# tgale96/sputnik

Hardware: AMD Instinct MI355X
Metric: effective TFLOP/s (nnz-FLOPs) DSD block=128 M=K=N=4096 @ 1/2/4/8 GPU vs density (higher is better)
Workload: dtype f16

## Files before the change

sputnik_amd/csrc/dispatch.cpp:

```cpp
#include <algorithm>
#include <cstdint>
#include <mutex>

#include "api_internal.h"
#include "block_gemm.h"
#include "dispatch_internal.h"
#include "dsd4w.h"
#include "metadata.h"
#include "sputnik/sputnik.h"
#include "sputnik_amd.h"

namespace sputnik_amd {

static unsigned long long *g_debug = nullptr;

static bool PairsEnabled() {
#ifdef SPUTNIK_NO_PAIRS
  return false;
#endif
  return Knob(kKnobPairs) != 0;
}

#ifndef SPUTNIK_PAIR_MIN_MEAN4
#define SPUTNIK_PAIR_MIN_MEAN4 8
// ... 421 lines not shown
  if (out == OutMode::kAccF32) p.c_ld *= 2;
  if (!acc) p.xcd_rows = Knob(kKnobXcdRows);
  PreparePairs(&p, blocks, stream, dry, !acc);
  GemmParams t = p;
  r->tall = UseTall(&t);
  if (r->tall && !acc && !dds && UseTallPipe(p, blocks, row_max, ta, tb)) {
    p.persistent = 0;
    p.num_jtiles = p.j_limit / 512;
    p.tall_flush_w = Knob(kKnobTallFlushW);
    p.tall_odd_share = Knob(kKnobTallOddShare);
    int dev = 0;
    p.num_tiles = hipGetDevice(&dev) == hipSuccess ? DeviceCUs(dev) : 0;
    r->code = 4;
    r->epi = 7;
    return;
  }
  if (r->tall) {
    p = t;
    BindTileCounter(&p, stream, dry);
  }
  const long long blocks4w = Dsd4wForced() ? (1LL << 40) : blocks;
  if (acc || !Dsd4wEnabled() ||
      !(dds ? Dds4wApplies(p, blocks4w, tb, !ta, true, r->tall)
            : Dsd4wApplies(p, blocks4w, !ta, tb, false, r->tall))) {
    r->code = r->tall ? 2 : p.pair != 0 && p.pair_split > 1 ? 3 : 0;
    return;
  }
  r->code = 1;
  r->epi = Dsd4wEpi();
  if (dds) {
    if (p.pair_xcd2 != 0) p.pair_xcd2 = Knob(kKnobDdsXcd2);
  } else if (Knob(kKnobDsd4w) == 1 && blocks < 12LL * p.num_rows) {
    r->epi = 5;
  }
}

constexpr long long kDsdBtMinRatio = 15000;
static bool BtAppliesDsd(const BlockMatrix &a, bool ta, const Matrix &b, bool tb) {
  if (!tb || ta || !BtGate(b)) return false;
  const long long blocks = a.nonzeros / (kBlock * kBlock);
  return blocks * 16384 >= kDsdBtMinRatio * b.cols;
}

static DenseRoute RouteDsd(const BlockMatrix &a, bool ta, const Matrix &b, bool tb,
                           const Matrix &c, hipStream_t stream, OutMode out, bool dry,
                           BtView view) {
  DenseRoute r;
  r.status = PrepareDsd(a, ta, b, tb, c, &r.p, &r.needs_meta);
  if (r.status != Status::kOk) return r;
  r.bt = out == OutMode::kStore && view != BtView::kOff && BtAppliesDsd(a, ta, b, tb) &&
         BtViewOpen(view, stream);
  if (!r.bt)
    RouteDenseOut(&r, false, a.nonzeros / (kBlock * kBlock),
                  ((long long)a.cols + kBlock - 1) / kBlock, ta, tb, stream, out, dry);
  return r;
}

static DenseRoute RouteDds(const Matrix &a, bool ta, const BlockMatrix &b, bool tb,
                           const Matrix &c, hipStream_t stream, OutMode out, bool dry) {
  DenseRoute r;
  r.status = PrepareDds(a, ta, b, tb, c, &r.p, &r.needs_meta);
  if (r.status == Status::kOk)
    RouteDenseOut(&r, true, b.nonzeros / (kBlock * kBlock), 0, ta, tb, stream, out, dry);
  return r;
}

// ... 408 lines not shown
```

sputnik_amd/csrc/dsd4w.h:

```cpp
#ifndef SPUTNIK_AMD_DSD4W_H_
#define SPUTNIK_AMD_DSD4W_H_

#include <hip/hip_runtime.h>

#include "block_gemm.h"

namespace sputnik_amd {

constexpr int kDsd4wMinMean = 2;
bool Dsd4wApplies(const GemmParams &p, long long blocks, bool s_kc, bool d_kc,
                  bool out_t, bool tall);

hipError_t LaunchDsd4w(int dtype, const GemmParams &p, int epi, bool nt,
                       hipStream_t stream, bool tn = false, bool tt = false);
constexpr int kDsd4wDefaultEpi = 3;

bool Dds4wApplies(const GemmParams &p, long long blocks, bool s_kc, bool d_kc,
                  bool out_t, bool tall);
hipError_t LaunchDds4w(int dtype, const GemmParams &p, int epi, bool nt,
                       hipStream_t stream, bool tn = false, bool tt = false);

bool Sdd4wApplies(const GemmParams &p, bool grouped, bool ta, bool tb, long long blocks = -1);
hipError_t LaunchSdd4w(int dtype, const GemmParams &p, bool ta, bool tb, int epi,
                       hipStream_t stream);

}

#endif
```

sputnik_amd/csrc/dsd4w.hip:

```cpp
#include <hip/hip_runtime.h>
#include <stdint.h>

#include <cstdlib>

#include "api_internal.h"
#include "block_gemm.h"
#include "dsd4w.h"
#include "dsd4w_asm.inc"

namespace sputnik_amd {
namespace {

constexpr int kRankScratch = 24576;
constexpr uint32_t kOob = 0x80000000u;

struct Pick {
  int row_a, row_b, e_a, n_a, e_b, n_b, target;
  int uniform;
};

__device__ Pick rank_wave(const GemmParams &p, char *lds, int wave, int lane,
                          int ra, int rb, int o0_pre, bool pre) {
  const int R = p.num_rows;
  const int o0 = pre ? o0_pre : lane <= R ? p.s_offsets[lane] : 0;
  const int o1 = __shfl_down(o0, 1, 64);
  const int nr = lane < R ? o1 - o0 : -1;
  int *keys = reinterpret_cast<int *>(lds + kRankScratch + wave * 256);
  int *nbr = reinterpret_cast<int *>(lds + kRankScratch + 2048 + wave * 256);
  const bool live = lane < R;
  const int key = live ? (nr << 6) | (63 - lane) : -1;
  keys[lane] = key;
  int4 k4[16];
#pragma unroll
  for (int j = 0; j < 16; ++j) k4[j] = *reinterpret_cast<const int4 *>(keys + 4 * j);
  int rank = 0;
#pragma unroll
  for (int j = 0; j < 16; ++j)
    rank += (k4[j].x > key) + (k4[j].y > key) + (k4[j].z > key) + (k4[j].w > key);
  const unsigned long long ba = __ballot(live && rank == ra);
  const unsigned long long bb = __ballot(live && rank == rb);
  Pick out;
// ... 49 lines not shown
    const int v = i == j ? n_by_rank[i] : (n_by_rank[i] + n_by_rank[j] + 1) / 2;
    atomicMax(&scratch[2], v);
  }
  __syncthreads();
  Pick out;
  out.row_a = __builtin_amdgcn_readfirstlane(scratch[0]);
  out.row_b = __builtin_amdgcn_readfirstlane(scratch[1]);
  out.target = __builtin_amdgcn_readfirstlane(scratch[2]);
  out.uniform = __builtin_amdgcn_readfirstlane(scratch[3]);
  out.e_a = __builtin_amdgcn_readfirstlane(offs[out.row_a]);
  out.n_a = __builtin_amdgcn_readfirstlane(offs[out.row_a + 1]) - out.e_a;
  out.e_b = __builtin_amdgcn_readfirstlane(offs[out.row_b]);
  out.n_b = __builtin_amdgcn_readfirstlane(offs[out.row_b + 1]) - out.e_b;
  __syncthreads();
  return out;
}

__device__ __forceinline__ unsigned long long exp_stamp(int dep) {
#if (SPUTNIK_EXP & 512) != 0
  unsigned long long t;
  asm volatile("s_memrealtime %0\n s_waitcnt lgkmcnt(0)"
               : "=s"(t) : "s"(__builtin_amdgcn_readfirstlane(dep)));
  return t;
#else
  (void)dep;
  return 0;
#endif
}

template <bool kBf16, int kEpi, bool kDds, bool kSdd = false, bool kNt = false,
          bool kTt = false, bool kTn = false>
__global__ void __launch_bounds__(256, 1) dsd4w_kernel(const GemmParams p) {
  constexpr bool kWaveEpi = kEpi != 0;
  constexpr bool kDs = kEpi == 3 || kEpi == 4 || kEpi == 5 || kEpi == 6 || kEpi == 7;
  constexpr bool kBar2 = kEpi == 4;
  constexpr bool kKs = kEpi == 6;
  constexpr bool kTp = kEpi == 7;
  static_assert(!kTp || (!kSdd && !kDds && !kNt && !kTt && !kTn), "tall pipeline: DSD NN");
  static_assert(!kDds || kEpi == 1 || kEpi == 3, "DDS: per-wave epilogue only");
  static_assert(!kSdd || ((kEpi == 3 || (kEpi == 4 && !kTt) || (kEpi == 1 && kTn) ||
                           (kKs && !kNt && !kTt && !kTn)) && !kDds),
                "SDD: double slots (TN: per-step images), per-wave epilogue");
  static_assert(!kKs || kSdd, "K-split: SDD NN only");
  constexpr bool kARowsT = (kTt || kTn) && kSdd;
  constexpr bool kDdsTt = kDds && kTt;
  [[maybe_unused]] const unsigned long long t_entry = __builtin_amdgcn_s_memrealtime();
  __shared__ __attribute__((aligned(1024))) char lds[163840];
  const int tid = threadIdx.x;
  const int lane = tid & 63;
  const int wave = __builtin_amdgcn_readfirstlane(tid >> 6);
  const uint32_t lbase =
      (uint32_t)(uintptr_t)((__attribute__((address_space(3))) char *)lds);

  constexpr int kIdxPreload = 1024;
  const int nb_all = p.s_blocks;
  [[maybe_unused]] const unsigned long long t_karg = exp_stamp(nb_all);
  const bool idx_pre = nb_all <= kIdxPreload &&
                       (reinterpret_cast<uintptr_t>(p.s_indices) & 15) == 0;
  typedef unsigned v4u_t __attribute__((ext_vector_type(4)));
  v4u_t idx_lo = {0u, 0u, 0u, 0u}, idx_hi = {0u, 0u, 0u, 0u};
  if (idx_pre) {
    const __amdgpu_buffer_rsrc_t ri = __builtin_amdgcn_make_buffer_rsrc(
        const_cast<short *>(p.s_indices), 0, (nb_all * 2 + 3) & ~3, 0x00020000);
    idx_lo = __builtin_bit_cast(v4u_t, __builtin_amdgcn_raw_buffer_load_b128(
                                            ri, lane * 32, 0, 0));
    idx_hi = __builtin_bit_cast(v4u_t, __builtin_amdgcn_raw_buffer_load_b128(
                                            ri, lane * 32 + 16, 0, 0));
// ... 725 lines not shown
    } else if constexpr (kSdd && kBar2) {
      if constexpr (kBf16)
        asm volatile(DSD4W_ASM_BF16_W3_SDD : DSD4W_OPERANDS_W : DSD4W_CLOBBERS);
      else
        asm volatile(DSD4W_ASM_F16_W3_SDD : DSD4W_OPERANDS_W : DSD4W_CLOBBERS);
    } else if constexpr (kSdd) {
      if constexpr (kBf16)
        asm volatile(DSD4W_ASM_BF16_W2_SDD : DSD4W_OPERANDS_W : DSD4W_CLOBBERS);
      else
        asm volatile(DSD4W_ASM_F16_W2_SDD : DSD4W_OPERANDS_W : DSD4W_CLOBBERS);
    } else if constexpr (kDds && kDs && (SPUTNIK_EXP & 512) != 0) {
      const unsigned long long t_asm = __builtin_amdgcn_s_memrealtime();
      unsigned long long r0 = 0, r1 = 0, r2 = 0, r3 = 0, r4 = 0;
      if constexpr (kBf16)
        asm volatile(DSD4W_ASM_BF16_W2_DDS_T : [r0] "=&s"(r0), [r1] "=&s"(r1),
                     [r2] "=&s"(r2), [r3] "=&s"(r3), [r4] "=&s"(r4)
                     : DSD4W_INPUTS_W : DSD4W_CLOBBERS);
      else
        asm volatile(DSD4W_ASM_F16_W2_DDS_T : [r0] "=&s"(r0), [r1] "=&s"(r1),
                     [r2] "=&s"(r2), [r3] "=&s"(r3), [r4] "=&s"(r4)
                     : DSD4W_INPUTS_W : DSD4W_CLOBBERS);
      DSD4W_RECORD((unsigned long long)((collect ? 2 : 0) | (producer ? 1 : 0)), 0ull);
    } else if constexpr (kDds && kDs) {
      if constexpr (kBf16)
        asm volatile(DSD4W_ASM_BF16_W2_DDS : DSD4W_OPERANDS_W : DSD4W_CLOBBERS);
      else
        asm volatile(DSD4W_ASM_F16_W2_DDS : DSD4W_OPERANDS_W : DSD4W_CLOBBERS);
    } else if constexpr (kDds) {
      if constexpr (kBf16)
        asm volatile(DSD4W_ASM_BF16_W_DDS : DSD4W_OPERANDS_W : DSD4W_CLOBBERS);
      else
        asm volatile(DSD4W_ASM_F16_W_DDS : DSD4W_OPERANDS_W : DSD4W_CLOBBERS);
    } else if constexpr ((SPUTNIK_EXP & 512) != 0 &&
                         (kEpi == 1 || kEpi == 3 || kEpi == 5)) {
      const unsigned long long t_asm = __builtin_amdgcn_s_memrealtime();
      unsigned long long r0 = 0, r1 = 0, r2 = 0, r3 = 0, r4 = 0;
#define DSD4W_STAMPED(NAME)                                                    \
  asm volatile(NAME : [r0] "=&s"(r0), [r1] "=&s"(r1), [r2] "=&s"(r2),          \
               [r3] "=&s"(r3), [r4] "=&s"(r4)                                  \
               : DSD4W_INPUTS_W : DSD4W_CLOBBERS)
      if constexpr (kEpi == 5) {
        if constexpr (kBf16) DSD4W_STAMPED(DSD4W_ASM_BF16_W4_T);
        else DSD4W_STAMPED(DSD4W_ASM_F16_W4_T);
      } else if constexpr (kEpi == 3) {
        if constexpr (kBf16) DSD4W_STAMPED(DSD4W_ASM_BF16_W2_T);
        else DSD4W_STAMPED(DSD4W_ASM_F16_W2_T);
      } else {
        if constexpr (kBf16) DSD4W_STAMPED(DSD4W_ASM_BF16_W_T);
        else DSD4W_STAMPED(DSD4W_ASM_F16_W_T);
      }
#undef DSD4W_STAMPED
      DSD4W_RECORD((unsigned long long)((collect ? 2 : 0) | (producer ? 1 : 0)), 0ull);
    } else if constexpr (kEpi == 5) {
      if constexpr (kBf16)
        asm volatile(DSD4W_ASM_BF16_W4 : DSD4W_OPERANDS_W : DSD4W_CLOBBERS);
      else
        asm volatile(DSD4W_ASM_F16_W4 : DSD4W_OPERANDS_W : DSD4W_CLOBBERS);
    } else if constexpr (kBar2) {
      if constexpr (kBf16)
        asm volatile(DSD4W_ASM_BF16_W3 : DSD4W_OPERANDS_W : DSD4W_CLOBBERS);
      else
        asm volatile(DSD4W_ASM_F16_W3 : DSD4W_OPERANDS_W : DSD4W_CLOBBERS);
    } else if constexpr (kDs) {
      if constexpr (kBf16)
        asm volatile(DSD4W_ASM_BF16_W2 : DSD4W_OPERANDS_W : DSD4W_CLOBBERS);
      else
        asm volatile(DSD4W_ASM_F16_W2 : DSD4W_OPERANDS_W : DSD4W_CLOBBERS);
    } else if constexpr (kEpi == 2) {
      if constexpr (kBf16)
        asm volatile(DSD4W_ASM_BF16_WL : DSD4W_OPERANDS_W : DSD4W_CLOBBERS);
      else
        asm volatile(DSD4W_ASM_F16_WL : DSD4W_OPERANDS_W : DSD4W_CLOBBERS);
    } else if constexpr (kWaveEpi) {
      if constexpr (kBf16)
        asm volatile(DSD4W_ASM_BF16_W : DSD4W_OPERANDS_W : DSD4W_CLOBBERS);
      else
        asm volatile(DSD4W_ASM_F16_W : DSD4W_OPERANDS_W : DSD4W_CLOBBERS);
    } else {
      if constexpr (kBf16)
        asm volatile(DSD4W_ASM_BF16 : DSD4W_OPERANDS_G : DSD4W_CLOBBERS);
      else
        asm volatile(DSD4W_ASM_F16 : DSD4W_OPERANDS_G : DSD4W_CLOBBERS);
      __syncthreads();
      for (int id = tid; id < 128 * 64; id += 256) {
        const int r = id >> 6, cc = id & 63;
// ... 66 lines not shown

hipError_t LaunchDsd4w(int dtype, const GemmParams &p, int epi, bool nt,
                       hipStream_t stream, bool tn, bool tt) {
  if (p.num_tiles <= 0) return hipSuccess;
  const dim3 grid(p.pair_split == 2 ? p.grid : p.num_tiles), block(256);
  if (tt) {
    if (dtype == 1)
      hipLaunchKernelGGL((dsd4w_kernel<true, 3, false, false, false, true>), grid, block, 0,
                         stream, p);
    else
      hipLaunchKernelGGL((dsd4w_kernel<false, 3, false, false, false, true>), grid, block, 0,
                         stream, p);
    return hipGetLastError();
  }
  if (tn) {
    if (dtype == 1)
      hipLaunchKernelGGL((dsd4w_kernel<true, 1, false, false, false, false, true>), grid,
                         block, 0, stream, p);
    else
      hipLaunchKernelGGL((dsd4w_kernel<false, 1, false, false, false, false, true>), grid,
                         block, 0, stream, p);
    return hipGetLastError();
  }
  if (nt) {
    if (dtype == 1)
      hipLaunchKernelGGL((dsd4w_kernel<true, 3, false, false, true>), grid, block, 0, stream, p);
    else
      hipLaunchKernelGGL((dsd4w_kernel<false, 3, false, false, true>), grid, block, 0, stream, p);
    return hipGetLastError();
  }
#define DSD4W_LAUNCH(B, E) \
  hipLaunchKernelGGL((dsd4w_kernel<B, E, false>), grid, block, 0, stream, p)
  if (dtype == 1) {
    if (epi == 7) DSD4W_LAUNCH(true, 7);
    else if (epi == 5) DSD4W_LAUNCH(true, 5);
    else if (epi == 4) DSD4W_LAUNCH(true, 4);
    else if (epi == 3) DSD4W_LAUNCH(true, 3);
    else if (epi == 2) DSD4W_LAUNCH(true, 2);
    else if (epi == 1) DSD4W_LAUNCH(true, 1);
    else DSD4W_LAUNCH(true, 0);
  } else {
    if (epi == 7) DSD4W_LAUNCH(false, 7);
    else if (epi == 5) DSD4W_LAUNCH(false, 5);
    else if (epi == 4) DSD4W_LAUNCH(false, 4);
    else if (epi == 3) DSD4W_LAUNCH(false, 3);
    else if (epi == 2) DSD4W_LAUNCH(false, 2);
    else if (epi == 1) DSD4W_LAUNCH(false, 1);
    else DSD4W_LAUNCH(false, 0);
  }
#undef DSD4W_LAUNCH
  return hipGetLastError();
}

bool Dds4wApplies(const GemmParams &p, long long blocks, bool s_kc, bool d_kc,
                  bool out_t, bool tall) {
  return out_t && !tall && (s_kc || p.s_block_offsets != nullptr) &&
         (p.pair_split <= 1 || (p.pair_split == 2 && p.split_bn == 512)) &&
         p.persistent == 0 && p.num_rows <= kLptRows &&
         CfgSparse::kBN == 512 && p.j_limit % 128 == 0 &&
         blocks >= (long long)kDsd4wMinMean * p.num_rows;
}

hipError_t LaunchDds4w(int dtype, const GemmParams &p, int epi, bool nt,
                       hipStream_t stream, bool tn, bool tt) {
  if (p.num_tiles <= 0) return hipSuccess;
  const dim3 grid(p.pair_split == 2 ? p.grid : p.num_tiles), block(256);
  if (tt) {
    if (dtype == 1)
      hipLaunchKernelGGL((dsd4w_kernel<true, 3, true, false, false, true>), grid, block, 0,
                         stream, p);
    else
      hipLaunchKernelGGL((dsd4w_kernel<false, 3, true, false, false, true>), grid, block, 0,
                         stream, p);
    return hipGetLastError();
  }
// ... 84 lines not shown
```

sputnik_amd/csrc/gen_dsd4w.py:

```python
import sys

FS = (128, 192)
FD = (160, 224)
SLOT = 8192
DMA_POS = [3, 9, 15, 21, 27, 33, 39, 45, 51, 57]
READS_AT = 2
NAN_F16 = "0x7e007e00"
NAN_BF16 = "0x7fc07fc0"
WAIT_TICKS = 20000000


def mfma(dt, m, n, s, zero_c=False):
    a = 4 * (8 * m + n)
    c = "0" if zero_c else f"a[{a}:{a + 3}]"
    return (f"v_mfma_f32_16x16x32_{dt} a[{a}:{a + 3}], "
            f"v[{FD[s] + 4 * n}:{FD[s] + 4 * n + 3}], "
            f"v[{FS[s] + 4 * m}:{FS[s] + 4 * m + 3}], {c}")


def d_reads(slot, s, into=None):
    out = []
    for n in range(8):
        b = (into or FD)[s] + 4 * n
        out.append(f"ds_read_b64_tr_b16 v[{b}:{b + 1}], %[vrd{n}] offset:{slot * SLOT}")
        out.append(f"ds_read_b64_tr_b16 v[{b + 2}:{b + 3}], %[vrd{n}] "
                   f"offset:{slot * SLOT + 1024}")
    return out


def t_reads(slot, s):
    out = []
    for m in range(8):
        b = FS[s] + 4 * m
        out.append(f"ds_read_b64_tr_b16 v[{b}:{b + 1}], %[vrt{m}] offset:{slot * SLOT}")
        out.append(f"ds_read_b64_tr_b16 v[{b + 2}:{b + 3}], %[vrt{m}] "
                   f"offset:{slot * SLOT + 1024}")
    return out


def s_reads(slot, s):
    return [f"ds_read_b128 v[{FS[s] + 4 * m}:{FS[s] + 4 * m + 3}], %[vrs] "
            f"offset:{slot * SLOT + m * 1024}" for m in range(8)]


def dmas(slot):
    out = []
    for q in range(2):
        out.append((f"s_add_u32 m0, %[ms], {slot * SLOT + q * 1024}",
                    f"buffer_load_dwordx4 %[vs], s[40:43], {'0' if q == 0 else 's72'} "
                    f"offen lds"))
    for q in range(8):
        out.append((f"s_add_u32 m0, %[md], {slot * SLOT + q * 1024}",
                    f"buffer_load_dwordx4 %[vd{(q >> 1) & 1}], s[44:47], s{64 + q} "
                    f"offen lds"))
    return out


VARIANT = {"dds": False, "ds": False, "sdd": False, "nt": False, "tt": False,
           "bar2": False, "tn": False, "ddstt": False, "il": False, "ks": False,
           "tp": False}


def col_order():
    if VARIANT["ddstt"]:
        return False
    return ((VARIANT["dds"] and not VARIANT["nt"])
            or ((VARIANT["tn"] or VARIANT["tt"]) and not VARIANT["sdd"]))


def a_rows_t():
    return (VARIANT["tt"] or VARIANT["tn"]) and VARIANT["sdd"]


def s_block_shift():
    return (24, 8) if VARIANT["sdd"] else (17, 15)


def advance():
    s = ("%[sk32]" if a_rows_t() else
         8192 if VARIANT["dds"] or VARIANT["tn"] else 64)
    return [f"s_add_u32 s40, s40, {s}", "s_addc_u32 s41, s41, 0",
            "s_add_u32 s44, s44, %[k32]", "s_addc_u32 s45, s45, 0"]


def entry_of(xreg, out_reg):
    if VARIANT["tp"]:
        tmp = "s77" if out_reg == "s76" else "s76"
        return ["s_nop 3", f"v_readlane_b32 {out_reg}, %[vent], {xreg}",
                f"v_readlane_b32 {tmp}, %[vent2], {xreg}", f"s_cmp_lt_u32 {xreg}, 64",
                f"s_cselect_b32 {out_reg}, {out_reg}, {tmp}",
                f"s_and_b32 {out_reg}, {out_reg}, 0xffffff"]
    return [f"s_cmp_lt_u32 {xreg}, %[n1]",
            f"s_cselect_b32 {out_reg}, %[b1], %[b2m]",
# ... 334 lines not shown
    k = 2 * (n_odd + n_even)
    check = [f"s_waitcnt vmcnt({k})", "v_readfirstlane_b32 s98, v97",
             "s_cmp_eq_u32 s98, %[epoch]", "s_cbranch_scc0 L_loop_%="]
    loads1 = []
    for f in range(8):
        loads1 += [(4 + 2 * f, x) for x in _pload(f)]
    loads3 = []
    for f in range(8, 24):
        loads3 += [(8 + 2 * (f - 8), x) for x in _pload(f)]
    body = step_ds(dt, 0)
    body += step_ds(dt, 1, wait=n_even, stores=loads1, no_dma=True)
    body += step_ds(dt, 2, wait=8, no_dma=True)
    body += step_ds(dt, 3, wait=-1, stores=loads3, no_dma=True, no_reads=True)
    return flag_load, check, body


def epilogue_collect_pre(cvt):
    out = []
    for f in range(24, 32):
        out += _pload(f)
    for i in range(64):
        t = 224 + 8 * (i % 4)
        out += [f"v_accvgpr_read_b32 v{t + j}, a{4 * i + j}" for j in range(4)]
        out.append(f"s_waitcnt vmcnt({min(31, 63 - i)})")
        p = 96 + 4 * (i % 32)
        out += [f"v_add_f32 v{t + j}, v{t + j}, v{p + j}" for j in range(4)]
        if i + 32 < 64:
            out += _pload(i + 32)
        out += [f"{cvt} v{t + 4}, v{t}, v{t + 1}", f"{cvt} v{t + 5}, v{t + 2}, v{t + 3}",
                f"ds_write_b64 %[vws{i % 8}], v[{t + 4}:{t + 5}] offset:{4096 * (i // 8)}"]
    return out


def prologue_ds():
    out = prologue_setup()

    def issue(pairs):
        r = []
        for m0, ld in pairs:
            r += [m0, "s_nop 0", ld]
        return r
    own_ds = own_ds_dmas if VARIANT["nt"] else (lambda d: [])
    out += issue(per_step_dmas(0)) + advance_per_step()
    out += issue(ds_dmas(0)) + issue(own_ds(0)) + advance_ds()
    out += issue(per_step_dmas(1)) + advance_per_step()
    out += [f"s_waitcnt vmcnt({ds_counts()[1]})", "s_barrier"]
    if VARIANT["ddstt"]:
        out += t_reads(0, 0) + own_reads_kc(0, 0, 0)
    elif VARIANT["nt"]:
        out += own_reads_kc(0, 0, 0) + s_reads_ds(0, 0, 0)
    elif VARIANT["tt"]:
        out += own_reads_kc(0, 0, 0) + d_reads(0, 0, FS)
    else:
        out += d_reads(0, 0) + s_reads_ds(0, 0, 0)
    out += issue(per_step_dmas(2)) + advance_per_step()
    out += issue(ds_dmas(1)) + issue(own_ds(1))
    out.append("s_waitcnt lgkmcnt(0)")
    return out


def convert(cvt, i):
    t = 96 + 8 * (i % 4)
    m, n = i // 8, i % 8
    out = [f"v_accvgpr_read_b32 v{t + j}, a{4 * i + j}" for j in range(4)]
    out += [f"{cvt} v{t + 4}, v{t}, v{t + 1}", f"{cvt} v{t + 5}, v{t + 2}, v{t + 3}",
            f"ds_write_b64 %[vws{n}], v[{t + 4}:{t + 5}] offset:{4096 * m}"]
# ... 76 lines not shown
        base = "%[vw0]" if m < 4 else "%[vw1]"
        off = 16 * (m % 4) * 1040 + 32 * n
        return f"ds_write_b64 {base}, {src} offset:{off}"

    def load(i):
        v = 128 + 4 * (i % 32)
        return [f"s_mov_b32 s78, {(i // 4) * 4096}",
                f"buffer_load_dwordx4 v[{v}:{v + 3}], %[vpl], s[84:87], s78 offen "
                f"offset:{(i % 4) * 1024} sc1"]

    if mode == "nan":
        nan = NAN_F16 if cvt.endswith("f16_f32") else NAN_BF16
        out += [f"v_mov_b32 v96, {nan}", "v_mov_b32 v97, v96"]
        out += [stage(i, "v[96:97]") for i in range(64)]
        return out
    if mode == "collect":
        for i in range(32):
            out += load(i)
    for i in range(64):
        t = 96 + 8 * (i % 4)
        a = 4 * i
        out += [f"v_accvgpr_read_b32 v{t + j}, a{a + j}" for j in range(4)]
        if mode == "collect":
            out.append(f"s_waitcnt vmcnt({min(31, 63 - i)})")
            p = 128 + 4 * (i % 32)
            out += [f"v_add_f32 v{t + j}, v{t + j}, v{p + j}" for j in range(4)]
            if i + 32 < 64:
                out += load(i + 32)
        out += [f"{cvt} v{t + 4}, v{t}, v{t + 1}", f"{cvt} v{t + 5}, v{t + 2}, v{t + 3}"]
        out.append(stage(i, f"v[{t + 4}:{t + 5}]"))
    return out


def epilogue_plain_interleaved(cvt):
    out = ["s_mov_b32 s84, %[cdlo]", "s_mov_b32 s85, %[cdhi]",
           "s_mov_b32 s86, 0x7fffffff", "s_mov_b32 s87, 0x00020000",
           "s_mov_b32 s78, 0"]
    for m in range(8):
        for n in range(8):
            i = 8 * m + n
            t = 96 + 8 * (i % 4)
            out += [f"v_accvgpr_read_b32 v{t + j}, a{4 * i + j}" for j in range(4)]
            out += [f"{cvt} v{t + 4}, v{t}, v{t + 1}", f"{cvt} v{t + 5}, v{t + 2}, v{t + 3}",
                    f"ds_write_b64 %[vws{n}], v[{t + 4}:{t + 5}] offset:{4096 * m}"]
        base = 128 + 16 * (m % 2)
        for j in range(4):
            out.append(f"ds_read_b128 v[{base + 4 * j}:{base + 4 * j + 3}], "
                       f"%[vrb{j}] offset:{4096 * m}")
        out.append("s_waitcnt lgkmcnt(0)")
        for j in range(4):
            out += [f"buffer_store_dwordx4 v[{base + 4 * j}:{base + 4 * j + 3}], %[vco], "
                    f"s[84:87], s78 offen nt",
                    "s_add_u32 s78, s78, %[c4]"]
        out.append("s_nop 1")
    return out


def copy_out():
    out = ["s_waitcnt lgkmcnt(0)",
           "s_mov_b32 s84, %[cdlo]", "s_mov_b32 s85, %[cdhi]",
           "s_mov_b32 s86, 0x7fffffff", "s_mov_b32 s87, 0x00020000",
           "s_mov_b32 s78, 0"]
    for b in range(8):
        base = 96 + 16 * (b % 2)
        idx = [4 * b + j for j in range(4)]
        for j, i in enumerate(idx):
            out.append(f"ds_read_b128 v[{base + 4 * j}:{base + 4 * j + 3}], "
                       f"%[vrb{i % 4}] offset:{4096 * (i // 4)}")
        out.append("s_waitcnt lgkmcnt(0)")
        for j, i in enumerate(idx):
            out += [f"buffer_store_dwordx4 v[{base + 4 * j}:{base + 4 * j + 3}], %[vco], "
                    f"s[84:87], s78 offen nt",
                    "s_add_u32 s78, s78, %[c4]"]
        out.append("s_nop 1")
    return out


def poll():
    return ["s_memrealtime s[96:97]", "s_waitcnt lgkmcnt(0)",
            "L_poll_%=:",
            "v_mov_b32 v96, 0",
            "global_load_dword v97, v96, %[flag] sc1",
            "s_waitcnt vmcnt(0)", "s_nop 0",
            "v_readfirstlane_b32 s98, v97",
            "s_cmp_eq_u32 s98, %[epoch]", "s_cbranch_scc1 L_got_%=",
            "s_sleep 1",
            "s_memrealtime s[98:99]", "s_waitcnt lgkmcnt(0)",
            "s_sub_u32 s98, s98, s96", "s_subb_u32 s99, s99, s97",
            "s_cmp_lg_u32 s99, 0", "s_cbranch_scc1 L_timeout_%=",
            f"s_cmp_lt_u32 s98, {WAIT_TICKS}", "s_cbranch_scc1 L_poll_%=",
            "L_timeout_%=:",
            "s_bitcmp1_b32 %[flags], 4", "s_cbranch_scc0 L_nan_%=",
            "s_mov_b64 s[78:79], exec", "s_mov_b64 exec, 1",
            "v_mov_b32 v96, 0", "v_mov_b32 v97, 1",
            "global_atomic_add v96, v97, %[err]",
            "s_waitcnt vmcnt(0)",
            "s_mov_b64 exec, s[78:79]",
            "s_branch L_nan_%="]


TP_NO_STORES = [False]


def tall_flush(cvt, dt, stamps=False):
    out = ["L_tflush_%=:"]
    if stamps:
# ... 150 lines not shown
    b0, nb = 8 * g // S, 8 // S
    out += ["s_waitcnt lgkmcnt(0)",
            "s_mov_b32 s84, %[cdlo]", "s_mov_b32 s85, %[cdhi]",
            "s_mov_b32 s86, 0x7fffffff", "s_mov_b32 s87, 0x00020000",
            f"s_mul_i32 s78, %[c4], {4 * b0}"]
    for b in range(b0, b0 + nb):
        base = 96 + 16 * (b % 2)
        for j in range(4):
            out.append(f"ds_read_b128 v[{base + 4 * j}:{base + 4 * j + 3}], "
                       f"%[vrb{j}] offset:{4096 * b}")
        out.append("s_waitcnt lgkmcnt(0)")
        for j in range(4):
            out += [f"buffer_store_dwordx4 v[{base + 4 * j}:{base + 4 * j + 3}], %[vco], "
                    f"s[84:87], s78 offen nt",
                    "s_add_u32 s78, s78, %[c4]"]
        out.append("s_nop 1")
    out.append("s_branch L_fin_%=")
    return out


def ksplit():
    out = ["L_ks_%=:"]
    for S in KS_CHUNKS:
        for g in range(S):
            out += [f"s_cmp_eq_u32 %[kss], {S}", f"s_cbranch_scc0 L_ksn{S}_{g}_%=",
                    f"s_cmp_eq_u32 %[kch], {g}", f"s_cbranch_scc1 L_ks{S}_{g}_%=",
                    f"L_ksn{S}_{g}_%=:"]
    out.append("s_branch L_fin_%=")
    return out


def build(dt, wave_epi=False, last_block=False, stamps=False, dds=False, ds=False,
          sdd=False, nt=False, tt=False, bar2=False, tn=False, ddstt=False, il=False,
          ks=False, tp=False):
    VARIANT.update(dds=dds, ds=ds, sdd=sdd, nt=nt, tt=tt, bar2=bar2, tn=tn, ddstt=ddstt,
                   il=il, ks=ks, tp=tp)
    try:
        return _build(dt, wave_epi, last_block, stamps)
    finally:
        VARIANT.update(dds=False, ds=False, sdd=False, nt=False, tt=False, bar2=False,
                       tn=False, ddstt=False, il=False, ks=False, tp=False)


def _build(dt, wave_epi, last_block, stamps):
    cvt = f"v_cvt_pk_{dt}_f32"
    body = prologue()
    if VARIANT["tp"]:
        body.append("s_mov_b32 s90, 0")
    if stamps and VARIANT["tp"]:
        body += ["s_mov_b32 s88, 0", "s_mov_b32 s89, 0"]
    if stamps:
        body.append("s_memrealtime %[r0]")
    body.append("s_branch L_first_%=")
    early = VARIANT["ds"] and not VARIANT["bar2"] and not VARIANT["sdd"]
    body.append("L_loop_%=:")
    body += step(dt, 0)
    body.append("L_mid_%=:")
    for H in (1, 2, 3):
        if H == 2:
            body.append("L_s2_%=:")
        if H == 3:
            if early:
                body += ["s_cmp_eq_u32 s61, %[pubat]", "s_cbranch_scc1 L_pubs_%=",
                         "s_cmp_eq_u32 s61, %[publast]", "s_cbranch_scc1 L_publ_%="]
            body.append("L_s3_%=:")
        body += step(dt, H)
    if VARIANT["tp"]:
        body.append("L_blkend_%=:")
    body.append("s_sub_u32 s61, s61, 1")
    if VARIANT["tp"]:
        body += ["s_sub_u32 s74, %[ntot], s61", "s_sub_u32 s74, s74, 1", "s_nop 3",
                 "v_readlane_b32 s75, %[vtile], s74", "v_readlane_b32 s76, %[vtile2], s74",
                 "s_cmp_lt_u32 s74, 64", "s_cselect_b32 s75, s75, s76",
                 "s_bitcmp1_b32 s75, 31", "s_cbranch_scc1 L_tflush_%="]
    body += ["s_cmp_eq_u32 s61, %[flushrem]", "s_cbranch_scc1 L_pub_%="]
    if early:
        body += ["s_cmp_eq_u32 s61, %[clbf]", "s_cbranch_scc1 L_clbf_%=",
                 "s_cmp_eq_u32 s61, %[clbc]", "s_cbranch_scc1 L_clbc_%="]
    if last_block:
        body += ["s_cmp_eq_u32 s61, 1", "s_cbranch_scc0 L_cont_%=",
                 "s_bitcmp1_b32 %[flags], 1", "s_cbranch_scc1 L_last_%=",
                 "L_cont_%=:"]
    body += ["s_cmp_lg_u32 s61, 0", "s_cbranch_scc1 L_loop_%=",
             "s_branch L_exit_%="]
    if last_block:
        body.append("L_last_%=:")
        if stamps:
            body.append("s_memrealtime %[r1]")
        body += step(dt, 0)
        for H in (1, 2, 3):
            body += step(dt, H, last=H, cvt=cvt)
        body += ["s_nop 7", "s_nop 7"] + convert(cvt, 62) + convert(cvt, 63)
        body.append("s_branch L_done_%=")
    if early:
        seq, rejoin = publish_sequence(dt)
        body.append("L_pubs_%=:")
        body += seq
        body.append(f"s_branch {rejoin}")
        body.append("L_publ_%=:")
        body += publish_last(dt, stamps)
        body.append("s_branch L_zero_%=")
        flag_load, check, clb = consumer_last_block(dt)
        body.append("L_clbf_%=:")
        body += flag_load
        body.append("s_branch L_loop_%=")
        body.append("L_clbc_%=:")
        body += check
        body += clb
        if stamps:
            body.append("s_memrealtime %[r1]")
        body += ["s_nop 7", "s_nop 7"]
        body += epilogue_collect_pre(cvt)
        body.append("s_branch L_done_%=")
    body.append("L_pub_%=:")
    if stamps:
        body += ["s_memrealtime %[r3]", "s_waitcnt lgkmcnt(0)"]
    body += publish()
    if stamps:
        body += ["s_memrealtime %[r4]", "s_waitcnt lgkmcnt(0)"]
    body += ["s_cmp_eq_u32 s61, 0", "s_cbranch_scc1 L_zero_%="]
    body.append("L_first_%=:")
    body += step(dt, 0, zero_c=True)
    body.append("s_branch L_mid_%=")
    body.append("L_zero_%=:")
    body += ["s_bitcmp1_b32 %[flags], 5", "s_cbranch_scc1 L_fin_%="]
    body += [f"v_accvgpr_write_b32 a{i}, 0" for i in range(256)]
    body.append("L_exit_%=:")
    if stamps:
        body.append("s_memrealtime %[r1]")
    if wave_epi:
        body += ["s_waitcnt vmcnt(0)", "s_nop 7", "s_nop 7"]
    else:
        body += ["s_waitcnt vmcnt(0)", "s_barrier", "s_nop 7", "s_nop 7"]
    if VARIANT["ks"]:
        body += ["s_cmp_gt_u32 %[kss], 1", "s_cbranch_scc1 L_ks_%="]
    body += ["s_bitcmp1_b32 %[flags], 0", "s_cbranch_scc1 L_collect_%="]
    if VARIANT["bar2"] or VARIANT["il"]:
        body += epilogue_plain_interleaved(cvt)
        body.append("s_branch L_end_%=")
    else:
        body += epilogue_body(cvt, "plain", wave_epi)
        body.append("s_branch L_done_%=")
    body.append("L_collect_%=:")
    body += poll()
    body.append("L_got_%=:")
    body += epilogue_body(cvt, "collect", wave_epi)
# ... 70 lines not shown
        for name, dds, sdd in (("_W_TN", False, False), ("_W_DDS_TN", True, False),
                               ("_W_SDD_TN", False, True)):
            lines.append(f"#define DSD4W_ASM_{dt.upper()}{name} \\")
            lines += [f'  "{ins}\\n" \\'
                      for ins in build(dt, True, dds=dds, sdd=sdd, tn=True)]
            lines += ['  ""', ""]
        lines.append(f"#define DSD4W_ASM_{dt.upper()}_W2_DDS_TT \\")
        lines += [f'  "{ins}\\n" \\'
                  for ins in build(dt, True, dds=True, ds=True, ddstt=True)]
        lines += ['  ""', ""]
        lines.append(f"#define DSD4W_ASM_{dt.upper()}_W4 \\")
        lines += [f'  "{ins}\\n" \\' for ins in build(dt, True, ds=True, il=True)]
        lines += ['  ""', ""]
        for name, il in (("_W2_T", False), ("_W4_T", True)):
            lines.append(f"#define DSD4W_ASM_{dt.upper()}{name} \\")
            lines += [f'  "{ins}\\n" \\'
                      for ins in build(dt, True, False, True, ds=True, il=il)]
            lines += ['  ""', ""]
        for name, sdd, nt in (("_W3", False, False), ("_W3_SDD", True, False),
                              ("_W3_SDD_NT", True, True)):
            lines.append(f"#define DSD4W_ASM_{dt.upper()}{name} \\")
            lines += [f'  "{ins}\\n" \\'
                      for ins in build(dt, True, False, False, False, True, sdd, nt,
                                       False, True)]
            lines += ['  ""', ""]
    clob = ([f'"a{i}"' for i in range(256)] + [f'"v{i}"' for i in range(96, 256)]
            + [f'"s{i}"' for i in range(40, 48)] + [f'"s{i}"' for i in range(56, 80)]
            + [f'"s{i}"' for i in range(84, 91)] + [f'"s{i}"' for i in range(96, 100)]
            + ['"scc"', '"vcc"', '"memory"'])
    lines.append("#define DSD4W_CLOBBERS " + ", ".join(clob))
    return "\n".join(lines) + "\n"


def main():
    with open(sys.argv[1], "w") as f:
        f.write(render())


if __name__ == "__main__":
    main()
```

sputnik_amd/csrc/knobs.cpp:

```cpp
#include <atomic>
#include <cstdlib>
#include <cstring>
#include <mutex>

#include "api_internal.h"
#include "dsd4w.h"

namespace sputnik_amd {

struct KnobDef {
  const char *name;
  const char *env;
  int def, lo, hi;
};
static const KnobDef kKnobs[kNumKnobs] = {
    {"pairs", "SPUTNIK_AMD_PAIRS", 1, 0, 1},
    {"pair_xcd2", "SPUTNIK_AMD_PAIR_XCD2", 3, 0, 3},
    {"split", "SPUTNIK_AMD_SPLIT", 1, 0, 1},
    {"split_min_bn", "SPUTNIK_AMD_SPLIT_MIN_BN", 128, 0, 1 << 20},
    {"dsd4w", "SPUTNIK_AMD_DSD4W", 1, 0, 7},
    {"grouped_sdd", "SPUTNIK_AMD_GROUPED_SDD", 1, 0, 1},
    {"grouped_min_per_cu", "SPUTNIK_AMD_GROUPED_MIN_PER_CU", 4, 0, 1 << 20},
    {"tall", "SPUTNIK_AMD_TALL", 1, 0, 2},
    {"tall_persistent", "SPUTNIK_AMD_TALL_PERSISTENT", 1, 0, 1},
    {"dds_xcd2", "SPUTNIK_AMD_DDS_XCD2", 3, 0, 3},
    {"sdd4w_max_ld", "SPUTNIK_AMD_SDD4W_MAX_LD", 16384, 0, 1 << 30},
    {"pair_fault", "SPUTNIK_AMD_PAIR_FAULT", 0, 0, 1},
    {"sdd_ksplit", "SPUTNIK_AMD_SDD_KSPLIT", 1, 1, 8},
    {"sdd_ksplit_min_k", "SPUTNIK_AMD_SDD_KSPLIT_MIN_K", 6144, 512, 1 << 30},
    {"sdd_order", "SPUTNIK_AMD_SDD_ORDER", 1, 0, 4},
    {"tall4w", "SPUTNIK_AMD_TALL4W", 1, 0, 1},
    {"tall_flush_w", "SPUTNIK_AMD_TALL_FLUSH_W", 4, 0, 64},
    {"tall_odd_share", "SPUTNIK_AMD_TALL_ODD_SHARE", 120, 50, 200},
    {"min_handoff", "SPUTNIK_AMD_MIN_HANDOFF", 2, 1, 64},
    {"xcd_rows", "SPUTNIK_AMD_XCD_ROWS", 1, 0, 1},
    {"sdd_krot", "SPUTNIK_AMD_SDD_KROT", 0, 0, 4},
    {"sdd_spread", "SPUTNIK_AMD_SDD_SPREAD", 2, 0, 2},
    {"sdd_bt_min_mib", "SPUTNIK_AMD_SDD_BT_MIN_MIB", 256, 0, 1 << 20},
    {"sdd_tail_min_k", "SPUTNIK_AMD_SDD_TAIL_MIN_K", 8192, 0, 1 << 30},
    {"sdd_act_route", "SPUTNIK_AMD_SDD_ACT_ROUTE", 0, 0, 2},
};
constexpr int kKnobUnset = -0x7fffffff - 1;
static std::atomic<int> g_knobs[kNumKnobs];
static std::once_flag g_knobs_once;

static void InitKnobs() {
  std::call_once(g_knobs_once, [] {
    for (int i = 0; i < kNumKnobs; ++i) {
      const char *e = std::getenv(kKnobs[i].env);
      char *end = nullptr;
      const long v0 = e != nullptr && *e != 0 ? std::strtol(e, &end, 10) : 0;
      const bool ok = e != nullptr && *e != 0 && end != nullptr && *end == 0 &&
                      v0 >= kKnobs[i].lo && v0 <= kKnobs[i].hi;
// ... 4 lines not shown
}

int Knob(KnobId k) {
  InitKnobs();
  return g_knobs[k].load(std::memory_order_relaxed);
}

static int KnobIndex(const char *name) {
  if (name == nullptr) return -1;
  for (int i = 0; i < kNumKnobs; ++i)
    if (std::strcmp(name, kKnobs[i].name) == 0) return i;
  return -1;
}

int TuningGet(const char *name) {
  const int i = KnobIndex(name);
  return i < 0 ? kKnobUnset : Knob(static_cast<KnobId>(i));
}

int TuningSet(const char *name, int value) {
  const int i = KnobIndex(name);
  if (i < 0 || value < kKnobs[i].lo || value > kKnobs[i].hi) return kKnobUnset;
  InitKnobs();
  return g_knobs[i].exchange(value, std::memory_order_relaxed);
}

void SetPairFault(int on) { (void)TuningSet("pair_fault", on != 0 ? 1 : 0); }

static int Dsd4wMode() { return Knob(kKnobDsd4w); }
bool Dsd4wEnabled() { return Dsd4wMode() != 0; }
bool Dsd4wForced() { return Dsd4wMode() >= 2; }
int Dsd4wEpi() {
  const int m = Dsd4wMode();
  return m >= 2 ? m - 2 : kDsd4wDefaultEpi;
}
int SelectDsdKernel(int four_wave) {
  if (four_wave < 0) return Dsd4wMode();
  return TuningSet("dsd4w", four_wave > 7 ? 7 : four_wave);
}

}
```

Before: 1184.

## Add streamed DSD epilogue overlapping output conversion and stores with final MFMAs

Adds a new epilogue variant (epi 8) for the four-wave DSD kernel. In the last block it interleaves accumulator readback, f16/bf16 conversion, LDS staging and global stores into the MFMA schedule of the final K-step, instead of running them after the math finishes. A separate non-last-block path pre-interleaves collect adds with stores. Dispatch selects it automatically for dense-enough matrices (blocks >= 28 per row). The generator gains an lgkmcnt recount pass and store-less probe variants, which adds generator complexity and a risk of wait-count errors in the hand-scheduled asm.

```diff
diff --git a/sputnik_amd/csrc/dispatch.cpp b/sputnik_amd/csrc/dispatch.cpp
--- a/sputnik_amd/csrc/dispatch.cpp
+++ b/sputnik_amd/csrc/dispatch.cpp
@@ -477,6 +477,8 @@
     if (p.pair_xcd2 != 0) p.pair_xcd2 = Knob(kKnobDdsXcd2);
   } else if (Knob(kKnobDsd4w) == 1 && blocks < 12LL * p.num_rows) {
     r->epi = 5;
+  } else if (Knob(kKnobDsd4w) == 1 && blocks >= 28LL * p.num_rows) {
+    r->epi = kDsd4wStreamEpi;
   }
 }
 
diff --git a/sputnik_amd/csrc/dsd4w.h b/sputnik_amd/csrc/dsd4w.h
--- a/sputnik_amd/csrc/dsd4w.h
+++ b/sputnik_amd/csrc/dsd4w.h
@@ -14,6 +14,7 @@
 hipError_t LaunchDsd4w(int dtype, const GemmParams &p, int epi, bool nt,
                        hipStream_t stream, bool tn = false, bool tt = false);
 constexpr int kDsd4wDefaultEpi = 3;
+constexpr int kDsd4wStreamEpi = 8;
 
 bool Dds4wApplies(const GemmParams &p, long long blocks, bool s_kc, bool d_kc,
                   bool out_t, bool tall);
diff --git a/sputnik_amd/csrc/dsd4w.hip b/sputnik_amd/csrc/dsd4w.hip
--- a/sputnik_amd/csrc/dsd4w.hip
+++ b/sputnik_amd/csrc/dsd4w.hip
@@ -7,6 +7,7 @@
 #include "block_gemm.h"
 #include "dsd4w.h"
 #include "dsd4w_asm.inc"
+#include "dsd4w_stream_asm.inl"
 
 namespace sputnik_amd {
 namespace {
@@ -122,7 +123,10 @@
           bool kTt = false, bool kTn = false>
 __global__ void __launch_bounds__(256, 1) dsd4w_kernel(const GemmParams p) {
   constexpr bool kWaveEpi = kEpi != 0;
-  constexpr bool kDs = kEpi == 3 || kEpi == 4 || kEpi == 5 || kEpi == 6 || kEpi == 7;
+  constexpr bool kDs = kEpi == 3 || kEpi == 4 || kEpi == 5 || kEpi == 6 || kEpi == 7 ||
+                       kEpi == 8;
+  constexpr bool kStream = kEpi == 8;
+  static_assert(!kStream || (!kSdd && !kDds && !kNt && !kTt && !kTn), "streamed: DSD NN");
   constexpr bool kBar2 = kEpi == 4;
   constexpr bool kKs = kEpi == 6;
   constexpr bool kTp = kEpi == 7;
@@ -914,14 +918,20 @@
       else
         asm volatile(DSD4W_ASM_F16_W_DDS : DSD4W_OPERANDS_W : DSD4W_CLOBBERS);
     } else if constexpr ((SPUTNIK_EXP & 512) != 0 &&
-                         (kEpi == 1 || kEpi == 3 || kEpi == 5)) {
+                         (kEpi == 1 || kEpi == 3 || kEpi == 5 || kStream)) {
       const unsigned long long t_asm = __builtin_amdgcn_s_memrealtime();
       unsigned long long r0 = 0, r1 = 0, r2 = 0, r3 = 0, r4 = 0;
 #define DSD4W_STAMPED(NAME)                                                    \
   asm volatile(NAME : [r0] "=&s"(r0), [r1] "=&s"(r1), [r2] "=&s"(r2),          \
                [r3] "=&s"(r3), [r4] "=&s"(r4)                                  \
                : DSD4W_INPUTS_W : DSD4W_CLOBBERS)
-      if constexpr (kEpi == 5) {
+      if constexpr (kStream) {
+        if constexpr (kBf16) DSD4W_STAMPED(DSD4W_ASM_BF16_W5_T);
+        else DSD4W_STAMPED(DSD4W_ASM_F16_W5_T);
+      } else if constexpr ((SPUTNIK_EXP & 1024) != 0 && kEpi != 1) {
+        if constexpr (kEpi == 5) DSD4W_STAMPED(DSD4W_ASM_F16_W4_T_NS);
+        else DSD4W_STAMPED(DSD4W_ASM_F16_W2_T_NS);
+      } else if constexpr (kEpi == 5) {
         if constexpr (kBf16) DSD4W_STAMPED(DSD4W_ASM_BF16_W4_T);
         else DSD4W_STAMPED(DSD4W_ASM_F16_W4_T);
       } else if constexpr (kEpi == 3) {
@@ -933,6 +943,11 @@
       }
 #undef DSD4W_STAMPED
       DSD4W_RECORD((unsigned long long)((collect ? 2 : 0) | (producer ? 1 : 0)), 0ull);
+    } else if constexpr (kStream) {
+      if constexpr (kBf16)
+        asm volatile(DSD4W_ASM_BF16_W5 : DSD4W_OPERANDS_W : DSD4W_CLOBBERS);
+      else
+        asm volatile(DSD4W_ASM_F16_W5 : DSD4W_OPERANDS_W : DSD4W_CLOBBERS);
     } else if constexpr (kEpi == 5) {
       if constexpr (kBf16)
         asm volatile(DSD4W_ASM_BF16_W4 : DSD4W_OPERANDS_W : DSD4W_CLOBBERS);
@@ -1065,7 +1080,8 @@
 #define DSD4W_LAUNCH(B, E) \
   hipLaunchKernelGGL((dsd4w_kernel<B, E, false>), grid, block, 0, stream, p)
   if (dtype == 1) {
-    if (epi == 7) DSD4W_LAUNCH(true, 7);
+    if (epi == 8) DSD4W_LAUNCH(true, 8);
+    else if (epi == 7) DSD4W_LAUNCH(true, 7);
     else if (epi == 5) DSD4W_LAUNCH(true, 5);
     else if (epi == 4) DSD4W_LAUNCH(true, 4);
     else if (epi == 3) DSD4W_LAUNCH(true, 3);
@@ -1073,7 +1089,8 @@
     else if (epi == 1) DSD4W_LAUNCH(true, 1);
     else DSD4W_LAUNCH(true, 0);
   } else {
-    if (epi == 7) DSD4W_LAUNCH(false, 7);
+    if (epi == 8) DSD4W_LAUNCH(false, 8);
+    else if (epi == 7) DSD4W_LAUNCH(false, 7);
     else if (epi == 5) DSD4W_LAUNCH(false, 5);
     else if (epi == 4) DSD4W_LAUNCH(false, 4);
     else if (epi == 3) DSD4W_LAUNCH(false, 3);
diff --git a/sputnik_amd/csrc/gen_dsd4w.py b/sputnik_amd/csrc/gen_dsd4w.py
--- a/sputnik_amd/csrc/gen_dsd4w.py
+++ b/sputnik_amd/csrc/gen_dsd4w.py
@@ -1,3 +1,4 @@
+import re
 import sys
 
 FS = (128, 192)
@@ -58,7 +59,7 @@
 
 VARIANT = {"dds": False, "ds": False, "sdd": False, "nt": False, "tt": False,
            "bar2": False, "tn": False, "ddstt": False, "il": False, "ks": False,
-           "tp": False}
+           "tp": False, "st": False}
 
 
 def col_order():
@@ -459,6 +460,147 @@
     return out
 
 
+_VREG = re.compile(r"v\[(\d+):(\d+)\]|\bv(\d+)\b")
+
+
+def _vregs(text):
+    out = set()
+    for a, b, c in _VREG.findall(text):
+        out |= set(range(int(a), int(b) + 1)) if a else {int(c)}
+    return out
+
+
+def lgkm_recount(ins_list):
+    out, pending = [], []
+    for ins in ins_list:
+        op = ins.split(" ", 1)[0]
+        if op == "s_waitcnt" and "lgkmcnt(0)" in ins:
+            pending = []
+        regs = _vregs(ins)
+        hit = [k for k, w in enumerate(pending) if w & regs]
+        if hit:
+            n = len(pending) - 1 - hit[-1]
+            out.append(f"s_waitcnt lgkmcnt({min(n, 15)})")
+            pending = pending[hit[-1] + 1:]
+        out.append(ins)
+        if op.startswith("ds_read"):
+            pending.append(_vregs(ins.split(",", 1)[0]))
+        elif op.startswith("ds_write"):
+            pending.append(set())
+    return out
+
+
+ST_READBACK = ((112, 116, 120, 124), (128, 132, 192, 196))
+
+
+def stream_convert(cvt, m, n):
+    i = 8 * m + n
+    t = 96 + 8 * (n % 2)
+    rd = [f"v_accvgpr_read_b32 v{t + j}, a{4 * i + j}" for j in range(4)]
+    return (rd[:3],
+            [rd[3], f"{cvt} v{t + 4}, v{t}, v{t + 1}", f"{cvt} v{t + 5}, v{t + 2}, v{t + 3}",
+             f"ds_write_b64 %[vws{n}], v[{t + 4}:{t + 5}] offset:{4096 * (m % 2)}"])
+
+
+def stream_readback(m):
+    return [f"ds_read_b128 v[{r}:{r + 3}], %[vrb{j}] offset:{4096 * (m % 2)}"
+            for j, r in enumerate(ST_READBACK[m % 2])]
+
+
+def stream_stores(m):
+    return [[f"buffer_store_dwordx4 v[{r}:{r + 3}], %[vco], s[84:87], s78 offen nt",
+             "s_add_u32 s78, s78, %[c4]"] for r in ST_READBACK[m % 2]]
+
+
+def stream_last_block(dt, cvt, stamps=False):
+    out = step_ds(dt, 0)
+    s3 = s_reads_ds(1, 1, 1)
+    extra = [(g, s3[m]) for m, g in enumerate((27, 28, 31, 39, 47, 55))]
+    extra.append((62, "s_waitcnt vmcnt(0)"))
+    out += step_ds(dt, 1, wait=ds_counts()[1], stores=extra, no_dma=True)
+    gaps = [[] for _ in range(128)]
+    post = []
+    gaps[0] += ["s_mov_b32 s84, %[cdlo]", "s_mov_b32 s85, %[cdhi]",
+                "s_mov_b32 s86, 0x7fffffff", "s_mov_b32 s87, 0x00020000",
+                "s_mov_b32 s78, 0"]
+    d3 = d_reads(3, 1)
+    for n in range(8):
+        gaps[n] += d3[2 * n:2 * n + 2]
+    gaps[8].append(s3[6])
+    gaps[9].append(s3[7])
+
+    def at(g, ins):
+        (gaps[g] if g < 128 else post).extend(ins)
+    for m in range(7):
+        b = 16 * (m + 1)
+        for n in range(8):
+            first, second = stream_convert(cvt, m, n)
+            at(b + 2 * n, first)
+            at(b + 2 * n + 1, second)
+    if stamps:
+        post += ["s_memrealtime %[r1]", "s_waitcnt lgkmcnt(0)"]
+    for m in range(6):
+        b = 16 * (m + 2)
+        for j, rb in enumerate(stream_readback(m)):
+            at(b + j, [rb])
+        for j, st in enumerate(stream_stores(m)):
+            at(b + 6 + 3 * j, st)
+    post += stream_readback(6)
+    post += ["s_nop 7"] * 4
+    st6 = stream_stores(6)
+    for n in range(8):
+        first, second = stream_convert(cvt, 7, n)
+        post += first + second
+        if n % 2 == 1:
+            post += st6[n // 2]
+    post += stream_readback(7)
+    for st in stream_stores(7):
+        post += st
+    win = []
+    for p in range(128):
+        m, s, n = p // 16, (p // 8) % 2, p % 8
+        win.append(mfma(dt, m, n, s))
+        win += gaps[p]
+    return out + lgkm_recount(win + post)
+
+
+def epilogue_collect_pre_il(cvt):
+    out = ["s_mov_b32 s40, %[cdlo]", "s_mov_b32 s41, %[cdhi]",
+           "s_mov_b32 s42, 0x7fffffff", "s_mov_b32 s43, 0x00020000",
+           "s_mov_b32 s44, 0"]
+    vm = [f for f in range(24)]
+
+    def load(f):
+        vm.append(f)
+        return _pload(f)
+    for f in range(24, 32):
+        out += load(f)
+    for m in range(8):
+        for n in range(8):
+            i = 8 * m + n
+            t = 224 + 8 * (i % 2)
+            out += [f"v_accvgpr_read_b32 v{t + j}, a{4 * i + j}" for j in range(4)]
+            w = len(vm) - 1 - vm.index(i)
+            assert w <= 63, w
+            out.append(f"s_waitcnt vmcnt({w})")
+            p = 96 + 4 * (i % 32)
+            out += [f"v_add_f32 v{t + j}, v{t + j}, v{p + j}" for j in range(4)]
+            if i + 32 < 64:
+                out += load(i + 32)
+            out += [f"{cvt} v{t + 4}, v{t}, v{t + 1}", f"{cvt} v{t + 5}, v{t + 2}, v{t + 3}",
+                    f"ds_write_b64 %[vws{n}], v[{t + 4}:{t + 5}] offset:{4096 * m}"]
+        for j in range(4):
+            out.append(f"ds_read_b128 v[{240 + 4 * j}:{243 + 4 * j}], %[vrb{j}] "
+                       f"offset:{4096 * m}")
+        out.append("s_waitcnt lgkmcnt(0)")
+        for j in range(4):
+            out += [f"buffer_store_dwordx4 v[{240 + 4 * j}:{243 + 4 * j}], %[vco], "
+                    f"s[40:43], s44 offen nt",
+                    "s_add_u32 s44, s44, %[c4]"]
+            vm.append(-1)
+    return out
+
+
 def prologue_ds():
     out = prologue_setup()
 
@@ -601,6 +743,13 @@
     return out
 
 
+EPI_NO_STORES = [False]
+
+
+def _out_store(ins):
+    return [] if EPI_NO_STORES[0] else [ins]
+
+
 def epilogue_plain_interleaved(cvt):
     out = ["s_mov_b32 s84, %[cdlo]", "s_mov_b32 s85, %[cdhi]",
            "s_mov_b32 s86, 0x7fffffff", "s_mov_b32 s87, 0x00020000",
@@ -618,9 +767,9 @@
                        f"%[vrb{j}] offset:{4096 * m}")
         out.append("s_waitcnt lgkmcnt(0)")
         for j in range(4):
-            out += [f"buffer_store_dwordx4 v[{base + 4 * j}:{base + 4 * j + 3}], %[vco], "
-                    f"s[84:87], s78 offen nt",
-                    "s_add_u32 s78, s78, %[c4]"]
+            out += _out_store(f"buffer_store_dwordx4 v[{base + 4 * j}:{base + 4 * j + 3}], "
+                              f"%[vco], s[84:87], s78 offen nt")
+            out.append("s_add_u32 s78, s78, %[c4]")
         out.append("s_nop 1")
     return out
 
@@ -638,9 +787,9 @@
                        f"%[vrb{i % 4}] offset:{4096 * (i // 4)}")
         out.append("s_waitcnt lgkmcnt(0)")
         for j, i in enumerate(idx):
-            out += [f"buffer_store_dwordx4 v[{base + 4 * j}:{base + 4 * j + 3}], %[vco], "
-                    f"s[84:87], s78 offen nt",
-                    "s_add_u32 s78, s78, %[c4]"]
+            out += _out_store(f"buffer_store_dwordx4 v[{base + 4 * j}:{base + 4 * j + 3}], "
+                              f"%[vco], s[84:87], s78 offen nt")
+            out.append("s_add_u32 s78, s78, %[c4]")
         out.append("s_nop 1")
     return out
 
@@ -857,14 +1006,14 @@
 
 def build(dt, wave_epi=False, last_block=False, stamps=False, dds=False, ds=False,
           sdd=False, nt=False, tt=False, bar2=False, tn=False, ddstt=False, il=False,
-          ks=False, tp=False):
+          ks=False, tp=False, st=False):
     VARIANT.update(dds=dds, ds=ds, sdd=sdd, nt=nt, tt=tt, bar2=bar2, tn=tn, ddstt=ddstt,
-                   il=il, ks=ks, tp=tp)
+                   il=il, ks=ks, tp=tp, st=st)
     try:
         return _build(dt, wave_epi, last_block, stamps)
     finally:
         VARIANT.update(dds=False, ds=False, sdd=False, nt=False, tt=False, bar2=False,
-                       tn=False, ddstt=False, il=False, ks=False, tp=False)
+                       tn=False, ddstt=False, il=False, ks=False, tp=False, st=False)
 
 
 def _build(dt, wave_epi, last_block, stamps):
@@ -902,13 +1051,17 @@
     if early:
         body += ["s_cmp_eq_u32 s61, %[clbf]", "s_cbranch_scc1 L_clbf_%=",
                  "s_cmp_eq_u32 s61, %[clbc]", "s_cbranch_scc1 L_clbc_%="]
-    if last_block:
+    if last_block or VARIANT["st"]:
         body += ["s_cmp_eq_u32 s61, 1", "s_cbranch_scc0 L_cont_%=",
                  "s_bitcmp1_b32 %[flags], 1", "s_cbranch_scc1 L_last_%=",
                  "L_cont_%=:"]
     body += ["s_cmp_lg_u32 s61, 0", "s_cbranch_scc1 L_loop_%=",
              "s_branch L_exit_%="]
-    if last_block:
+    if VARIANT["st"]:
+        body.append("L_last_%=:")
+        body += stream_last_block(dt, cvt, stamps)
+        body.append("s_branch L_end_%=")
+    elif last_block:
         body.append("L_last_%=:")
         if stamps:
             body.append("s_memrealtime %[r1]")
@@ -935,8 +1088,12 @@
         if stamps:
             body.append("s_memrealtime %[r1]")
         body += ["s_nop 7", "s_nop 7"]
-        body += epilogue_collect_pre(cvt)
-        body.append("s_branch L_done_%=")
+        if VARIANT["st"]:
+            body += epilogue_collect_pre_il(cvt)
+            body.append("s_branch L_end_%=")
+        else:
+            body += epilogue_collect_pre(cvt)
+            body.append("s_branch L_done_%=")
     body.append("L_pub_%=:")
     if stamps:
         body += ["s_memrealtime %[r3]", "s_waitcnt lgkmcnt(0)"]
@@ -1073,9 +1230,30 @@
     return "\n".join(lines) + "\n"
 
 
+def render_stream():
+    lines = ["// generated by sputnik_amd/csrc/gen_dsd4w.py --stream -- do not edit", ""]
+    for dt in ("f16", "bf16"):
+        for name, stamped in (("_W5", False), ("_W5_T", True)):
+            lines.append(f"#define DSD4W_ASM_{dt.upper()}{name} \\")
+            lines += [f'  "{ins}\\n" \\'
+                      for ins in build(dt, True, False, stamped, ds=True, il=True, st=True)]
+            lines += ['  ""', ""]
+    EPI_NO_STORES[0] = True
+    try:
+        for name, il in (("_W2_T_NS", False), ("_W4_T_NS", True)):
+            lines.append(f"#define DSD4W_ASM_F16{name} \\")
+            lines += [f'  "{ins}\\n" \\'
+                      for ins in build("f16", True, False, True, ds=True, il=il)]
+            lines += ['  ""', ""]
+    finally:
+        EPI_NO_STORES[0] = False
+    return "\n".join(lines) + "\n"
+
+
 def main():
-    with open(sys.argv[1], "w") as f:
-        f.write(render())
+    stream = sys.argv[1] == "--stream"
+    with open(sys.argv[2 if stream else 1], "w") as f:
+        f.write(render_stream() if stream else render())
 
 
 if __name__ == "__main__":
diff --git a/sputnik_amd/csrc/knobs.cpp b/sputnik_amd/csrc/knobs.cpp
--- a/sputnik_amd/csrc/knobs.cpp
+++ b/sputnik_amd/csrc/knobs.cpp
@@ -18,7 +18,7 @@
     {"pair_xcd2", "SPUTNIK_AMD_PAIR_XCD2", 3, 0, 3},
     {"split", "SPUTNIK_AMD_SPLIT", 1, 0, 1},
     {"split_min_bn", "SPUTNIK_AMD_SPLIT_MIN_BN", 128, 0, 1 << 20},
-    {"dsd4w", "SPUTNIK_AMD_DSD4W", 1, 0, 7},
+    {"dsd4w", "SPUTNIK_AMD_DSD4W", 1, 0, 8},
     {"grouped_sdd", "SPUTNIK_AMD_GROUPED_SDD", 1, 0, 1},
     {"grouped_min_per_cu", "SPUTNIK_AMD_GROUPED_MIN_PER_CU", 4, 0, 1 << 20},
     {"tall", "SPUTNIK_AMD_TALL", 1, 0, 2},
@@ -89,11 +89,11 @@
 bool Dsd4wForced() { return Dsd4wMode() >= 2; }
 int Dsd4wEpi() {
   const int m = Dsd4wMode();
-  return m >= 2 ? m - 2 : kDsd4wDefaultEpi;
+  return m == 8 ? kDsd4wStreamEpi : m >= 2 ? m - 2 : kDsd4wDefaultEpi;
 }
 int SelectDsdKernel(int four_wave) {
   if (four_wave < 0) return Dsd4wMode();
-  return TuningSet("dsd4w", four_wave > 7 ? 7 : four_wave);
+  return TuningSet("dsd4w", four_wave > 8 ? 8 : four_wave);
 }
 
 }
```

Result: no change. 1184 (-0.1%).
